# xandergos/terrain-diffusion

Hardware: NVIDIA H100
Metric: denoising steps/sec, 256^2 latent tiles, 30m U-Net (higher is better)
Workload: dtype bf16

## Files before the change

terrain_diffusion_b200/csrc/tdx_igemm.cu:

```cuda
#include "tdx_common.h"
#include "tdx_ptx.cuh"

namespace tdx {

constexpr int kTileH = 16, kTileW = 8;
constexpr int kPatchH = kTileH + 2, kPatchW = kTileW + 2;
constexpr int kKcBytes = kPatchH * kPatchW * 16;
constexpr int kAStageBytes = 8 * kKcBytes;
constexpr int kSA = 3;
constexpr int kMaxSB = 18;
constexpr int kWQ = 2;
constexpr int kEpiWarps = 4 * kWQ;
constexpr int kChunk = 32;
constexpr int kGroups = kChunk / 8;
constexpr int kThreads = 128 + 32 * kEpiWarps;
constexpr int kMaxSplit = 8;
constexpr int kSmemMisc = 14336;
constexpr int kSmemBudget = 227 * 1024;
constexpr int kStgLd = 132;

struct FastDiv {
  uint32_t d, magic;
};
static FastDiv make_fastdiv(int d) {
  FastDiv f;
  f.d = (uint32_t)d;
  f.magic = d <= 1 ? 0u : (uint32_t)(0xFFFFFFFFull / (uint32_t)d + 1ull);
  return f;
}
__device__ __forceinline__ uint32_t fdiv(uint32_t n, const FastDiv& f) { return f.d == 1 ? n : __umulhi(n, f.magic); }

struct IgemmParams {
  int nseg;
  int seg_chunks[3];
  int seg_taps[3];
  const __nv_bfloat16* B;
  int cout, nsplit;
  float inv_cout;
  int ncta;
  int SA;
  int SB;
  int b_stage_bytes;
  int resident;
  int bgroup;
  int ksplit;
  float* ws;
  int H, W, nimg, tiles_x, tiles_y, num_items;
  FastDiv fd_ks, fd_nsplit, fd_per, fd_tx, fd_ty;
  int dtx, dty, dimg;
  int stages_per_item;
  int epi;
  int cluster_stats;
  int xsplit;
  const float* cvec;
  const uint4* resid;
  int resid_spatial, resid_pnorm;
  float resid_scale, clip;
  TdxOutSpec out[3];
  float* rms_out;
  const float* resid_inv;
  unsigned long long* timeline;
  unsigned long long* trace;
};

__device__ __forceinline__ void stage_locate(const IgemmParams& p, int s, int& seg, int& ch, int& tap, int& taps) {
  int base = 0;
  for (seg = 0;; ++seg) {
    taps = p.seg_taps[seg];
    const int n = p.seg_chunks[seg] * taps;
    if (s < base + n || seg == p.nseg - 1) break;
    base += n;
  }
  ch = taps == 9 ? (s - base) / 9 : (s - base);
  tap = (s - base) - ch * taps;
}

#ifndef TDX_DEBUG_HOOKS
#define TDX_DEBUG_HOOKS 0
#endif
#if TDX_DEBUG_HOOKS
#define TDX_TRACE(slot, it)                                                                  \
  do {                                                                                       \
    if (p.trace && blockIdx.x == 0 && (it) < 16) p.trace[(it) * 8 + (slot)] = clock64();     \
  } while (0)
#else
#define TDX_TRACE(slot, it) do { } while (0)
#endif

struct TileWalk {
  int tx, ty, img;
  int dtx, dty, dimg;
  int split, kpart;
  __device__ __forceinline__ void init(const IgemmParams& p) {
    const uint32_t b = blockIdx.x;
    const uint32_t bk = fdiv(b, p.fd_ks);
    kpart = (int)(b - bk * p.fd_ks.d);
    split = (int)(bk - fdiv(bk, p.fd_nsplit) * p.fd_nsplit.d);
    const uint32_t t = fdiv(b, p.fd_per);
    const uint32_t t1 = fdiv(t, p.fd_tx);
    tx = (int)(t - t1 * p.fd_tx.d);
    const uint32_t t2 = fdiv(t1, p.fd_ty);
    ty = (int)(t1 - t2 * p.fd_ty.d);
    img = (int)t2;
    dtx = p.dtx;
    dty = p.dty;
    dimg = p.dimg;
  }
  __device__ __forceinline__ void next(const IgemmParams& p) {
    tx += dtx;
    int c = tx >= p.tiles_x ? 1 : 0;
    tx -= c ? p.tiles_x : 0;
    ty += dty + c;
    c = ty >= p.tiles_y ? 1 : 0;
    ty -= c ? p.tiles_y : 0;
    img += dimg + c;
  }
};
__device__ __forceinline__ void stage_range(const IgemmParams& p, int kpart, int& s0, int& s1) {
  s0 = (int)fdiv((uint32_t)(p.stages_per_item * kpart), p.fd_ks);
  s1 = (int)fdiv((uint32_t)(p.stages_per_item * (kpart + 1)), p.fd_ks);
}

__device__ __forceinline__ uint32_t cluster_ctarank() {
  uint32_t r;
  asm volatile("mov.u32 %0, %%cluster_ctarank;" : "=r"(r));
  return r;
}
__device__ __forceinline__ uint32_t map_to_cta(uint32_t local_smem_addr, uint32_t rank) {
  uint32_t r;
  asm volatile("mapa.shared::cluster.u32 %0, %1, %2;" : "=r"(r) : "r"(local_smem_addr), "r"(rank));
  return r;
}
__device__ __forceinline__ void st_cluster_f32(uint32_t addr, float v) {
  asm volatile("st.shared::cluster.f32 [%0], %1;" ::"r"(addr), "f"(v) : "memory");
}
__device__ __forceinline__ void mbar_arrive_cluster(uint32_t remote_bar_addr) {
  asm volatile("mbarrier.arrive.release.cluster.shared::cluster.b64 _, [%0];" ::"r"(remote_bar_addr) : "memory");
}
__device__ __forceinline__ bool mbar_try_wait_cluster(uint64_t* bar, uint32_t parity) {
  uint32_t ok;
  asm volatile(
      "{\n\t"
      ".reg .pred P;\n\t"
      "mbarrier.try_wait.parity.acquire.cluster.shared::cta.b64 P, [%1], %2;\n\t"
      "selp.b32 %0, 1, 0, P;\n\t"
      "}\n"
      : "=r"(ok)
      : "r"(smem_u32(bar)), "r"(parity)
      : "memory");
  return ok != 0;
}
__device__ __forceinline__ void cluster_sync_all() {
  asm volatile("barrier.cluster.arrive.release.aligned;\n\tbarrier.cluster.wait.acquire.aligned;" ::: "memory");
}

__device__ __forceinline__ void load_acc(const float* stg, int m, int col, float (&v)[kChunk]) {
#pragma unroll
  for (int i = 0; i < kChunk; ++i) v[i] = stg[(col + i) * kStgLd + m];
}

__device__ __forceinline__ float inv_rms(float sumsq, float inv_n) {
  float s;
  asm("sqrt.approx.f32 %0, %1;" : "=f"(s) : "f"(sumsq * inv_n));
  return __fdividef(1.0f, 1e-4f + s);
}

__device__ __forceinline__ void store_chunk(uint4* dst, uint32_t plane, int Wo, int kind, int spatial, bool active,
                                            const float (&v)[kChunk], float hs, float hsk) {
  uint4 u[kGroups];
  if (kind == TDX_OUT_RAW) {
#pragma unroll
    for (int g = 0; g < kGroups; ++g) {
      u[g].x = pack_bf16x2(v[g * 8 + 0], v[g * 8 + 1]);
      u[g].y = pack_bf16x2(v[g * 8 + 2], v[g * 8 + 3]);
      u[g].z = pack_bf16x2(v[g * 8 + 4], v[g * 8 + 5]);
      u[g].w = pack_bf16x2(v[g * 8 + 6], v[g * 8 + 7]);
    }
  } else {
#pragma unroll
    for (int g = 0; g < kGroups; ++g) {
      float w[8];
#pragma unroll
      for (int i = 0; i < 8; ++i) w[i] = mp_silu_scaled(v[g * 8 + i], hs, hsk);
      u[g].x = pack_bf16x2(w[0], w[1]);
      u[g].y = pack_bf16x2(w[2], w[3]);
      u[g].z = pack_bf16x2(w[4], w[5]);
      u[g].w = pack_bf16x2(w[6], w[7]);
    }
  }
  if (!active) return;
  if (spatial == TDX_SP_UP2) {
#pragma unroll
    for (int g = 0; g < kGroups; ++g) {
      uint4* d = dst + (size_t)g * plane;
      d[0] = u[g];
      d[1] = u[g];
      d[Wo] = u[g];
      d[Wo + 1] = u[g];
    }
  } else {
#pragma unroll
    for (int g = 0; g < kGroups; ++g) dst[(size_t)g * plane] = u[g];
  }
}

struct ConsumerRing {
  int sa, sb;
  uint32_t pha;
  uint32_t fmask;
};

template <int kN>
__device__ __forceinline__ void mma_item(const IgemmParams& p, const uint8_t* a_ring, const uint8_t* b_ring,
                                         uint64_t* a_full, uint64_t* a_empty, uint64_t* b_full, uint64_t* b_empty,
                                         ConsumerRing& r, int s0, int s1, bool steady, float* stg) {
  const int lane = threadIdx.x & 31, wl = (threadIdx.x >> 5) & 3, wg = (int)(threadIdx.x >> 7) - 1;
  float acc[kN / 2];
#pragma unroll
  for (int i = 0; i < kN / 2; ++i) acc[i] = 0.f;
  constexpr uint32_t b_lbo = kN * 16;
  const uint32_t a_base = smem_u32(a_ring) + wg * 8 * kPatchW * 16;
  const uint32_t b_base = smem_u32(b_ring);
  const bool deep = p.SB > 1 || p.resident;
  int pend_a = -1, pend_b = -1;
  auto release = [&](int a, int b) {
    __syncwarp();
    if (lane == 0) {
      if (b >= 0) mbar_arrive(&b_empty[b]);
      if (a >= 0) mbar_arrive(&a_empty[a]);
    }
  };
  for (int s = s0; s < s1;) {
    int seg, ch, tap0, taps;
    stage_locate(p, s, seg, ch, tap0, taps);
    const int tap1 = (taps - tap0 < s1 - s) ? taps : tap0 + (s1 - s);
    const int nt = tap1 - tap0;
    s += nt;
    mbar_wait(&a_full[r.sa], r.pha);
    const uint32_t a_stage = a_base + r.sa * kAStageBytes;
    unsigned long long tt = taps == 9 ? (0x16ad18b50820ull >> (5 * tap0)) : (unsigned long long)(kPatchW + 1);
    const int gsz = steady ? nt : p.bgroup;
    int t = 0;
    for (int g0 = 0; g0 < nt; g0 += gsz) {
      const int gn = nt - g0 < gsz ? nt - g0 : gsz;
      if (!steady) {
        mbar_wait(&b_full[r.sb], (r.fmask >> r.sb) & 1u);
        r.fmask ^= 1u << r.sb;
      }
      for (int k = 0; k < gn; ++k, ++t, tt >>= 5) {
        const uint32_t al = a_stage + (uint32_t)(tt & 31ull) * 16;
        const uint32_t bl = b_base + r.sb * p.b_stage_bytes;
        wgmma_fence();
#pragma unroll
        for (int j = 0; j < 4; ++j)
          wgmma_bf16<kN>(acc, make_smem_desc(al + j * 2 * kKcBytes, kKcBytes, kPatchW * 16),
                         make_smem_desc(bl + j * 2 * b_lbo, b_lbo, 128), 1u);
        wgmma_commit();
        const int rel_b = p.resident ? -1 : r.sb;
        const int rel_a = t == nt - 1 ? r.sa : -1;
        if (deep) {
          wgmma_wait<1>();
          release(pend_a, pend_b);
          pend_a = rel_a;
          pend_b = rel_b;
        } else {
          wgmma_wait<0>();
          release(rel_a, rel_b);
        }
        if (++r.sb == p.SB) r.sb = 0;
      }
    }
    if (++r.sa == p.SA) { r.sa = 0; r.pha ^= 1; }
  }
  wgmma_wait<0>();
  release(pend_a, pend_b);
  named_bar_sync(13, 32 * kEpiWarps);
  float* dst = stg + 64 * wg + 16 * wl + (lane >> 2);
#pragma unroll
  for (int j = 0; j < kN / 8; ++j)
#pragma unroll
    for (int i = 0; i < 2; ++i)
#pragma unroll
      for (int c = 0; c < 2; ++c) dst[(8 * j + 2 * (lane & 3) + c) * kStgLd + 8 * i] = acc[4 * j + 2 * i + c];
  named_bar_sync(13, 32 * kEpiWarps);
}

template <bool kCL, int kN>
__global__ void __launch_bounds__(kThreads, 1)
igemm_kernel(const __grid_constant__ CUtensorMap tm0, const __grid_constant__ CUtensorMap tm1,
             const __grid_constant__ CUtensorMap tm2, const __grid_constant__ IgemmParams p) {
  extern __shared__ __align__(1024) uint8_t smem[];
  const int ksplit_ = kCL ? p.ksplit : 1;
  const bool cstats_ = kCL && p.cluster_stats;
  uint8_t* a_ring = smem;
  uint8_t* b_ring = smem + p.SA * kAStageBytes;
  uint64_t* bars = reinterpret_cast<uint64_t*>(b_ring + p.SB * p.b_stage_bytes);
  uint64_t* a_full = bars;
  uint64_t* a_empty = a_full + kSA;
  uint64_t* b_full = a_empty + kSA;
  uint64_t* b_empty = b_full + kMaxSB;
  uint64_t* x_full = b_empty + kMaxSB;
  float* ssq = reinterpret_cast<float*>(bars) + 256;
  float* rss = ssq + 512;
  float* stot = rss + 512;
  float* xstat = stot + 128;
  float* stg = reinterpret_cast<float*>(reinterpret_cast<uint8_t*>(bars) + kSmemMisc);

  const int warp = __shfl_sync(0xffffffffu, threadIdx.x >> 5, 0);
  const int lane = threadIdx.x & 31;
#if TDX_DEBUG_HOOKS
  if (p.trace && blockIdx.x == 0 && threadIdx.x == 0) p.trace[126] = clock64();
  if (p.timeline && threadIdx.x == 0) {
    unsigned long long t;
    asm volatile("mov.u64 %0, %globaltimer;" : "=l"(t));
    atomicMin(p.timeline, t);
  }
#endif

  if (warp == 0 && elect_one()) {
    tma_prefetch_desc(&tm0);
    if (p.nseg > 1) tma_prefetch_desc(&tm1);
    if (p.nseg > 2) tma_prefetch_desc(&tm2);
  }
  if (warp == 2) {
    constexpr int kBars = 2 * kSA + 2 * kMaxSB + 2;
    static_assert(kBars <= 64, "two barriers per lane");
    const int x_full0 = 2 * kSA + 2 * kMaxSB;
#pragma unroll
    for (int k = 0; k < 2; ++k) {
      const int i = lane + 32 * k;
      if (i < kBars) {
        uint32_t count = 1;
        if ((i >= kSA && i < 2 * kSA) || (i >= 2 * kSA + kMaxSB && i < x_full0)) count = kEpiWarps;
        if (i >= x_full0) count = p.xsplit > 1 ? (uint32_t)(p.xsplit - 1) * 128u : 1u;
        mbar_init(&bars[i], count);
      }
    }
    fence_mbar_init();
  }
  __syncthreads();
  if (cstats_) cluster_sync_all();
#if TDX_DEBUG_HOOKS
  if (p.trace && blockIdx.x == 0 && threadIdx.x == 0) p.trace[127] = clock64();
#endif
  pdl_launch_dependents();

  if (warp == 0) {
    pdl_wait();
    int sa = 0;
    uint32_t ph = 0;
    int it = 0;
    TileWalk tw;
    tw.init(p);
    int s0, s1;
    stage_range(p, tw.kpart, s0, s1);
    for (int item = blockIdx.x; item < p.num_items; item += gridDim.x, ++it, tw.next(p)) {
      const int img = tw.img, Y0 = tw.ty * kTileH, X0 = tw.tx * kTileW;
      if (lane == 0) TDX_TRACE(0, it);
      for (int s = s0; s < s1;) {
        int seg, ch, tap, taps;
        stage_locate(p, s, seg, ch, tap, taps);
        const CUtensorMap* tm = seg == 0 ? &tm0 : (seg == 1 ? &tm1 : &tm2);
        mbar_wait(&a_empty[sa], ph ^ 1);
        if (elect_one()) {
          mbar_expect_tx(&a_full[sa], kAStageBytes);
          tma_load_4d(tm, &a_full[sa], a_ring + sa * kAStageBytes, (X0 - 1) * 8, Y0 - 1, ch * 8, img);
        }
        __syncwarp();
        if (++sa == p.SA) { sa = 0; ph ^= 1; }
        s += taps - tap;
      }
    }
    if (ksplit_ > 1) cluster_sync_all();
  } else if (warp == 1) {
    int sb = 0;
    uint32_t ph = 0;
    TileWalk tw;
    tw.init(p);
    const int split = tw.split;
    int st0, st1;
    stage_range(p, tw.kpart, st0, st1);
    for (int item = blockIdx.x; item < p.num_items; item += gridDim.x) {
      const uint8_t* bsrc = reinterpret_cast<const uint8_t*>(p.B) +
                            ((size_t)split * p.stages_per_item + st0) * p.b_stage_bytes;
      if (p.bgroup == 1) {
        for (int ks = 0; ks < st1 - st0; ++ks) {
          mbar_wait(&b_empty[sb], ph ^ 1);
          if (elect_one()) {
            mbar_expect_tx(&b_full[sb], p.b_stage_bytes);
            bulk_load_1d(bsrc + (size_t)ks * p.b_stage_bytes, &b_full[sb], b_ring + sb * p.b_stage_bytes,
                         p.b_stage_bytes);
          }
          __syncwarp();
          if (++sb == p.SB) { sb = 0; ph ^= 1; }
        }
        continue;
      }
      int ks = 0;
      for (int s = st0; s < st1;) {
        int seg, ch, tap0, taps;
        stage_locate(p, s, seg, ch, tap0, taps);
        const int nt = (taps - tap0 < st1 - s) ? taps - tap0 : st1 - s;
        int head = sb, gi = 0;
        for (int t = 0; t < nt; ++t) {
          if (!p.resident) mbar_wait(&b_empty[sb], ph ^ 1);
          const bool first = gi == 0;
          if (++gi == p.bgroup) gi = 0;
          if (first) head = sb;
          if (elect_one()) {
            uint64_t* full = &b_full[head];
            if (first) mbar_expect_tx(full, (uint32_t)(nt - t < p.bgroup ? nt - t : p.bgroup) * p.b_stage_bytes);
            bulk_load_1d(bsrc + (size_t)(ks + t) * p.b_stage_bytes, full, b_ring + sb * p.b_stage_bytes,
                         p.b_stage_bytes);
          }
          __syncwarp();
          if (++sb == p.SB) { sb = 0; ph ^= 1; }
        }
        ks += nt;
        s += nt;
      }
      if (p.resident) break;
    }
    if (ksplit_ > 1) cluster_sync_all();
  } else if (warp < 4) {
    if (ksplit_ > 1) cluster_sync_all();
  } else {
    pdl_wait();
    const int q = warp & 3;
    const int wq = (warp - 4) >> 2;
    const int m = q * 32 + lane;
    const int y = m >> 3, x = m & 7;
    const int C8 = p.cout >> 3;
    const bool need_norm = (p.epi & TDX_EPI_PNORM) || p.out[0].kind == TDX_OUT_PNORM_SILU ||
                           p.out[1].kind == TDX_OUT_PNORM_SILU || p.out[2].kind == TDX_OUT_PNORM_SILU ||
                           p.rms_out != nullptr;
    const uint32_t my_rank = cstats_ ? cluster_ctarank() : 0;
    TileWalk tw;
    tw.init(p);
    ConsumerRing ring = {0, 0, 0u, 0u};
    int s0, s1;
    stage_range(p, tw.kpart, s0, s1);
    const int ks = ksplit_, kpart = tw.kpart;
    const int slice = p.ncta / ks, sch = slice / kChunk;
    const int nchunks_all = p.ncta / kChunk;
    const int nchunks = sch;
    const int col0 = kpart * slice;
    const int chbase = tw.split * p.ncta + col0;
    const uint32_t plane = (uint32_t)(p.H * p.W);
    struct OffSpec {
      uint32_t istride, rowstep, colstep, tpart;
    };
    auto make_spec = [&](int spatial, uint32_t planes_per_img) -> OffSpec {
      OffSpec o;
      if (spatial == TDX_SP_DOWN2) {
        o.istride = planes_per_img * (plane >> 2);
        o.rowstep = (uint32_t)(kTileH / 2) * (uint32_t)(p.W >> 1);
        o.colstep = kTileW / 2;
        o.tpart = (uint32_t)((y >> 1) * (p.W >> 1) + (x >> 1));
      } else if (spatial == TDX_SP_UP2) {
        o.istride = planes_per_img * (plane << 2);
        o.rowstep = (uint32_t)(kTileH * 2) * (uint32_t)(p.W << 1);
        o.colstep = kTileW * 2;
        o.tpart = (uint32_t)((y << 1) * (p.W << 1) + (x << 1));
      } else {
        o.istride = planes_per_img * plane;
        o.rowstep = (uint32_t)kTileH * (uint32_t)p.W;
        o.colstep = kTileW;
        o.tpart = (uint32_t)(y * p.W + x);
      }
      return o;
    };
    auto item_off = [&](const OffSpec& o, const TileWalk& t) -> uint32_t {
      return (uint32_t)t.img * o.istride + (uint32_t)t.ty * o.rowstep + (uint32_t)t.tx * o.colstep + o.tpart;
    };
    const bool has_resid = (p.epi & TDX_EPI_RESID) != 0;
    const uint32_t rplane = p.resid_spatial == TDX_SP_UP2 ? (plane >> 2) : (p.resid_spatial == TDX_SP_DOWN2 ? (plane << 2) : plane);
    const int rsp = p.resid_spatial == TDX_SP_UP2 ? TDX_SP_DOWN2 : (p.resid_spatial == TDX_SP_DOWN2 ? TDX_SP_UP2 : TDX_SP_SAME);
    const OffSpec rspec = make_spec(rsp, (uint32_t)C8), rinv_spec = make_spec(rsp, 1u);
    OffSpec ospec[3];
    uint32_t omask = 0;
#pragma unroll
    for (int o = 0; o < 3; ++o) {
      const int sp = p.out[o].spatial;
      ospec[o] = make_spec(sp, (uint32_t)C8);
      const uint32_t oplane = sp == TDX_SP_DOWN2 ? (plane >> 2) : (sp == TDX_SP_UP2 ? (plane << 2) : plane);
      ospec[o].tpart += (uint32_t)(chbase >> 3) * oplane;
      omask |= (uint32_t)(p.out[o].kind != TDX_OUT_NONE && !(sp == TDX_SP_DOWN2 && ((y | x) & 1))) << o;
    }
    constexpr int kPreN = (kChunk / 4 > kGroups) ? kChunk / 4 : kGroups;
    uint4 pre[kPreN];
    const uint4* rbase_pre = nullptr;
    float rinv_pre = 1.f;
    const bool cv_ahead = (p.epi & TDX_EPI_EMB_SILU) && !has_resid;
    const bool ahead = has_resid || cv_ahead;
    const bool own_rnorm = has_resid && p.resid_pnorm && !p.resid_inv;
    auto fetch_ahead = [&](const TileWalk& t) {
      if (cv_ahead) {
        const uint4* cp = reinterpret_cast<const uint4*>(p.cvec + (size_t)t.img * p.cout + chbase + wq * kChunk);
#pragma unroll
        for (int j = 0; j < kChunk / 4; ++j) pre[j] = (wq < nchunks) ? __ldg(cp + j) : make_uint4(0, 0, 0, 0);
        return;
      }
      if (!has_resid) return;
      const int Y_ = t.ty * kTileH + y, X_ = t.tx * kTileW + x;
      const bool vld = (Y_ < p.H) && (X_ < p.W);
      rbase_pre = p.resid + item_off(rspec, t);
      if (p.resid_inv) rinv_pre = vld ? __ldg(p.resid_inv + item_off(rinv_spec, t)) : 0.f;
      const uint4* rptr = rbase_pre + (size_t)((chbase >> 3) + wq * kGroups) * rplane;
#pragma unroll
      for (int g = 0; g < kGroups; ++g)
        pre[g] = (vld && wq < nchunks) ? __ldg(rptr + (size_t)g * rplane) : make_uint4(0, 0, 0, 0);
    };
    if (ahead) fetch_ahead(tw);
    int it = 0;
    for (int item = blockIdx.x; item < p.num_items; item += gridDim.x, ++it, tw.next(p)) {
      const int img = tw.img;
      const int Y = tw.ty * kTileH + y, X = tw.tx * kTileW + x;
      const bool valid = (Y < p.H) && (X < p.W);
      if (warp == 4 && lane == 0) TDX_TRACE(1, it);
      mma_item<kN>(p, a_ring, b_ring, a_full, a_empty, b_full, b_empty, ring, s0, s1, p.resident && it > 0, stg);
      if (warp == 4 && lane == 0) TDX_TRACE(2, it);

      const float* red_src = nullptr;
      if (ks > 1) {
        float* wsg = p.ws + (size_t)fdiv((uint32_t)item, p.fd_ks) * (ks - 1) * p.ncta * 128;
        if (warp == 4 && lane == 0) TDX_TRACE(3, it);
        for (int ck = wq; ck < nchunks_all; ck += kWQ) {
          const int dst = ck / sch;
          if (dst == kpart) continue;
          const int slot = kpart - (kpart > dst ? 1 : 0);
          float* d = wsg + ((size_t)(dst * (ks - 1) + slot) * slice + (size_t)(ck - dst * sch) * kChunk) * 128 + m;
          float v[kChunk];
          __syncwarp();
          load_acc(stg, m, ck * kChunk, v);
#pragma unroll
          for (int j = 0; j < kChunk; ++j) __stcg(d + (size_t)j * 128, v[j]);
        }
        cluster_sync_all();
        red_src = wsg + (size_t)kpart * (ks - 1) * slice * 128 + m;
      }
      const float* cvb = p.cvec ? p.cvec + (size_t)img * p.cout + chbase : nullptr;
      auto add_partials = [&](int ck, float (&v)[kChunk]) {
        for (int kp = 0; kp < ks - 1; ++kp) {
          const float* src = red_src + ((size_t)kp * slice + (size_t)(ck * kChunk)) * 128;
#pragma unroll
          for (int j = 0; j < kChunk; ++j) v[j] += __ldcg(src + (size_t)j * 128);
        }
      };

      {
        float rscale = p.resid_scale;
        const uint4* rbase = rbase_pre;
        const bool more = ahead && item + (int)gridDim.x < p.num_items;
        TileWalk tn = tw;
        tn.next(p);
        if (has_resid && p.resid_inv) {
          rscale = p.resid_scale * rinv_pre;
        } else if (own_rnorm) {
          float ss = 0.f;
          auto sq8 = [&](const uint4& u) {
            float a, b;
            unpack_bf16x2(u.x, a, b); ss = fmaf(a, a, fmaf(b, b, ss));
            unpack_bf16x2(u.y, a, b); ss = fmaf(a, a, fmaf(b, b, ss));
            unpack_bf16x2(u.z, a, b); ss = fmaf(a, a, fmaf(b, b, ss));
            unpack_bf16x2(u.w, a, b); ss = fmaf(a, a, fmaf(b, b, ss));
          };
          if (valid) {
            for (int g0 = wq * 2; g0 < C8; g0 += 2 * kWQ) {
              const uint4 u0 = __ldg(rbase + (size_t)g0 * rplane), u1 = __ldg(rbase + (size_t)(g0 + 1) * rplane);
              sq8(u0);
              sq8(u1);
            }
          }
          rss[wq * 128 + m] = ss;
          named_bar_sync(9 + q, 32 * kWQ);
          ss = 0.f;
#pragma unroll
          for (int w = 0; w < kWQ; ++w) ss += rss[w * 128 + m];
          rscale = p.resid_scale * inv_rms(ss, p.inv_cout);
        }
        uint4* optr[3];
        bool oact[3];
#pragma unroll
        for (int o = 0; o < 3; ++o) {
          oact[o] = valid && ((omask >> o) & 1u);
          optr[o] = reinterpret_cast<uint4*>(p.out[o].ptr) + item_off(ospec[o], tw);
        }


        auto compute_v = [&](int ck, float (&v)[kChunk]) {
          __syncwarp();
          load_acc(stg, m, col0 + ck * kChunk, v);
          add_partials(ck, v);
          if (p.epi & TDX_EPI_EMB_SILU) {
#pragma unroll
            for (int i = 0; i < kChunk; i += 4) {
              const uint4 cu = (cv_ahead && ck == wq) ? pre[i >> 2] : __ldg(reinterpret_cast<const uint4*>(cvb + ck * kChunk + i));
              const float4 c4 = make_float4(__uint_as_float(cu.x), __uint_as_float(cu.y), __uint_as_float(cu.z), __uint_as_float(cu.w));
              v[i + 0] = mp_silu_f(v[i + 0] * c4.x);
              v[i + 1] = mp_silu_f(v[i + 1] * c4.y);
              v[i + 2] = mp_silu_f(v[i + 2] * c4.z);
              v[i + 3] = mp_silu_f(v[i + 3] * c4.w);
            }
          }
          if (p.epi & TDX_EPI_RESID) {
            const uint4* rptr = rbase + (size_t)((chbase >> 3) + ck * kGroups) * rplane;
#pragma unroll
            for (int g = 0; g < kGroups; ++g) {
              uint4 u = (ck == wq) ? pre[g] : (valid ? __ldg(rptr + (size_t)g * rplane) : make_uint4(0, 0, 0, 0));
              float rr[8];
              unpack_bf16x2(u.x, rr[0], rr[1]);
              unpack_bf16x2(u.y, rr[2], rr[3]);
              unpack_bf16x2(u.z, rr[4], rr[5]);
              unpack_bf16x2(u.w, rr[6], rr[7]);
#pragma unroll
              for (int i = 0; i < 8; ++i) v[g * 8 + i] = fmaf(rscale, rr[i], v[g * 8 + i]);
            }
          }
          if (p.clip > 0.f) {
#pragma unroll
            for (int i = 0; i < kChunk; ++i) v[i] = fminf(fmaxf(v[i], -p.clip), p.clip);
          }
        };
        auto emit_v = [&](int ck, float (&v)[kChunk], float inv) {
          if (p.epi & TDX_EPI_PNORM) {
#pragma unroll
            for (int i = 0; i < kChunk; ++i) v[i] *= inv;
          }
#pragma unroll
          for (int o = 0; o < 3; ++o) {
            const int kind = p.out[o].kind, sp = p.out[o].spatial;
            if (kind == TDX_OUT_NONE) continue;
            float hs = 0.5f * p.out[o].scale;
            if (kind == TDX_OUT_PNORM_SILU) hs = (p.epi & TDX_EPI_PNORM) ? 0.5f : 0.5f * inv;
            const uint32_t oplane = sp == TDX_SP_DOWN2 ? (plane >> 2) : (sp == TDX_SP_UP2 ? (plane << 2) : plane);
            const int Wo = sp == TDX_SP_DOWN2 ? (p.W >> 1) : (sp == TDX_SP_UP2 ? (p.W << 1) : p.W);
            store_chunk(optr[o] + (size_t)(ck * kGroups) * oplane, oplane, Wo, kind, sp, oact[o], v, hs,
                        hs * (1.0f / 0.596f));
          }
        };
        auto finish_norm = [&](float sumsq) -> float {
          ssq[wq * 128 + m] = sumsq;
          named_bar_sync(1 + q, 32 * kWQ);
          float tot = 0.f;
#pragma unroll
          for (int w = 0; w < kWQ; ++w) tot += ssq[w * 128 + m];
          if (cstats_) {
            const int par = it & 1;
            if (wq == 0) {
              for (uint32_t r = 0; r < (uint32_t)p.xsplit; ++r) {
                if (r == my_rank) continue;
                st_cluster_f32(map_to_cta(smem_u32(&xstat[(par * kMaxSplit + my_rank) * 128 + m]), r), tot);
                mbar_arrive_cluster(map_to_cta(smem_u32(&x_full[par]), r));
              }
              const uint32_t xph = (it >> 1) & 1;
              if (!mbar_try_wait_cluster(&x_full[par], xph)) {
                const long long t0 = clock64();
                while (!mbar_try_wait_cluster(&x_full[par], xph)) {
                  if (clock64() - t0 > TDX_WAIT_LIMIT) asm volatile("trap;");
                }
              }
              for (uint32_t r = 0; r < (uint32_t)p.xsplit; ++r)
                if (r != my_rank) tot += xstat[(par * kMaxSplit + r) * 128 + m];
              stot[m] = tot;
            }
            named_bar_sync(5 + q, 32 * kWQ);
            tot = stot[m];
          }
          return inv_rms(tot, p.inv_cout);
        };

        float v[kChunk];
        float sumsq = 0.f, inv = 1.f;
        const bool reuse = need_norm && nchunks <= kWQ;
#pragma unroll 1
        for (int pass = need_norm ? 0 : 1; pass < 2; ++pass) {
#pragma unroll 1
          for (int ck = wq; ck < nchunks; ck += kWQ) {
            if (pass == 0 || !reuse) {
              compute_v(ck, v);
              if (ck == wq && (reuse || pass == 1) && more) fetch_ahead(tn);
            }
            if (pass == 0) {
#pragma unroll
              for (int i = 0; i < kChunk; ++i) sumsq = fmaf(v[i], v[i], sumsq);
            } else {
              emit_v(ck, v, inv);
            }
          }
          if (pass == 0) {
            inv = finish_norm(sumsq);
            if (p.rms_out && wq == 0 && kpart == 0 && tw.split == 0 && valid)
              p.rms_out[(uint32_t)img * plane + (uint32_t)(Y * p.W + X)] = inv;
          }
        }
      }
      if (warp == 4 && lane == 0) TDX_TRACE(4, it);
    }
  }

  __syncthreads();
  if (cstats_) cluster_sync_all();
#if TDX_DEBUG_HOOKS
  if (p.trace && blockIdx.x == 0 && threadIdx.x == 96) p.trace[125] = clock64();
  if (p.timeline && threadIdx.x == 0) {
    unsigned long long t;
    asm volatile("mov.u64 %0, %globaltimer;" : "=l"(t));
    atomicMax(p.timeline + 1, t);
  }
#endif
}

static unsigned long long* g_trace_ptr = nullptr;
static unsigned long long* g_timeline_ptr = nullptr;
static int g_timeline_idx = 0, g_timeline_cap = 0;

static int ensure_scratch(float** ws);

typedef decltype(&igemm_kernel<false, 64>) IgemmKernel;

static IgemmKernel igemm_kernel_for(bool cluster, int n) {
  switch (n) {
    case 64: return cluster ? igemm_kernel<true, 64> : igemm_kernel<false, 64>;
    case 128: return cluster ? igemm_kernel<true, 128> : igemm_kernel<false, 128>;
    case 192: return cluster ? igemm_kernel<true, 192> : igemm_kernel<false, 192>;
    default: return cluster ? igemm_kernel<true, 256> : igemm_kernel<false, 256>;
  }
}

int igemm_prepare() {
  static bool seen[16] = {false};
  if (first_use_on_device(seen)) {
    for (int n = 64; n <= 256; n += 64)
      for (int cl = 0; cl < 2; ++cl)
        TDX_CHECK_CUDA(
            cudaFuncSetAttribute(igemm_kernel_for(cl, n), cudaFuncAttributeMaxDynamicSharedMemorySize, kSmemBudget));
  }
  float* ws;
  return ensure_scratch(&ws);
}

static bool needs_norm(const TdxIgemmDesc& d) {
  if (d.epi_flags & TDX_EPI_PNORM) return true;
  if (d.rms_out) return true;
  for (int o = 0; o < 3; ++o)
    if (d.out[o].kind == TDX_OUT_PNORM_SILU) return true;
  return false;
}

constexpr size_t kWsBytes = 24u << 20;
static float* g_ws[16] = {nullptr};

static int ensure_scratch(float** ws) {
  int dev = 0;
  TDX_CHECK_CUDA(cudaGetDevice(&dev));
  TDX_REQUIRE(dev >= 0 && dev < 16, "igemm: device index %d out of range", dev);
  if (!g_ws[dev]) TDX_CHECK_CUDA(cudaMalloc(&g_ws[dev], kWsBytes));
  *ws = g_ws[dev];
  return TDX_OK;
}

static int max_active_clusters(int csize) {
  static int cache[9] = {0};
  if (csize <= 1) return sm_count();
  if (csize > 8) return 0;
  if (cache[csize]) return cache[csize];
  cudaLaunchConfig_t cfg;
  memset(&cfg, 0, sizeof(cfg));
  cudaLaunchAttribute attr[1];
  cfg.gridDim = dim3((sm_count() / csize) * csize);
  cfg.blockDim = dim3(kThreads);
  cfg.dynamicSmemBytes = kSmemBudget;
  attr[0].id = cudaLaunchAttributeClusterDimension;
  attr[0].val.clusterDim.x = csize;
  attr[0].val.clusterDim.y = 1;
  attr[0].val.clusterDim.z = 1;
  cfg.attrs = attr;
  cfg.numAttrs = 1;
  int n = 0;
  cudaFuncSetAttribute(igemm_kernel<true, 64>, cudaFuncAttributeMaxDynamicSharedMemorySize, kSmemBudget);
  if (cudaOccupancyMaxActiveClusters(&n, igemm_kernel<true, 64>, &cfg) != cudaSuccess || n <= 0) {
    cudaGetLastError();
    n = (sm_count() * 3 / 4) / csize;
  }
  cache[csize] = n;
  return n;
}

struct ItemShape { int ncta, resident, sa, sb, ksplit; };

static ItemShape choose_item_shape(int cout, int tiles, int stages, int chunks, int forced_n, bool norm) {
  if (forced_n && (forced_n > cout || cout % forced_n)) forced_n = 0;
  double best = 1e30;
  ItemShape bs = {64, 0, kSA, 2, 1};
  for (int n = 64; n <= 256 && n <= cout; n += 64) {
    if (cout % n) continue;
    if (forced_n && n != forced_n) continue;
    const int nsplit = cout / n;
    if (norm && nsplit > kMaxSplit) continue;
    const int stage_bytes = n * 128;
    const int free_bytes = kSmemBudget - kSmemMisc - n * kStgLd * 4;
    const int sa = free_bytes - kSA * kAStageBytes >= 2 * stage_bytes ? kSA : 2;
    const int ring_budget = free_bytes - sa * kAStageBytes;
    const long items = (long)tiles * nsplit;
    for (int ks = 1; ks <= 8; ++ks) {
      const int csize = ks * ((norm && nsplit > 1) ? nsplit : 1);
      if (ks > 1) {
        if (n % (kChunk * ks) || ks > stages || csize > kMaxSplit) continue;
        if (items * ks > (long)max_active_clusters(csize) * csize) continue;
        if ((size_t)items * (ks - 1) * n * 512 > kWsBytes) continue;
      }
      const int my_stages = (stages + ks - 1) / ks;
      const int my_chunks = (chunks + ks - 1) / ks + (ks > 1 ? 1 : 0);
      const int resident = (ks == 1 && stages * stage_bytes <= ring_budget && stages <= kMaxSB) ? 1 : 0;
      int sb = resident ? stages : ring_budget / stage_bytes;
      if (sb > kMaxSB) sb = kMaxSB;
      if (sb < 1) continue;
      int grid = items * ks < sm_count() ? (int)(items * ks) : sm_count();
      grid -= grid % (nsplit * ks);
      if (grid <= 0) continue;
      const double rounds = (double)((items * ks + grid - 1) / grid);
      const double mma = rounds * my_stages * 4.0 * n * (sb < 2 && !resident ? 2.0 : 1.0) + 800.0;
      const double a_bytes = (double)items * ks * my_chunks * kAStageBytes;
      const double b_bytes = resident ? (double)grid * stages * stage_bytes : (double)items * stages * stage_bytes;
      const double red_bytes = ks > 1 ? (double)(ks - 1) / ks * n * 512.0 : 0.0;
      const double l2 = (a_bytes + b_bytes + 2.0 * red_bytes * items * ks) / 5000.0;
      const double per_sm = (double)(my_chunks * kAStageBytes + my_stages * stage_bytes) / 56.0;
      const int epi_chunks = ((n / ks) / kChunk + 3) / 4;
      const double epi = rounds * epi_chunks * 100.0;
      const double red = ks > 1 ? 2.0 * red_bytes / 56.0 + 2000.0 : 0.0;
      double t = mma;
      if (l2 > t) t = l2;
      if (per_sm > t) t = per_sm;
      t += epi + red;
      if (t < best) { best = t; bs = {n, resident, sa, sb, ks}; }
    }
  }
  return bs;
}

int igemm_launch(const TdxIgemmDesc& d, const CUtensorMap* tms, cudaStream_t stream) {
  IgemmParams p;
  memset(&p, 0, sizeof(p));
  p.nseg = d.n_seg;
  p.stages_per_item = 0;
  int chunks = 0;
  for (int s = 0; s < d.n_seg; ++s) {
    p.seg_chunks[s] = d.a_channels[s] / 64;
    p.seg_taps[s] = d.a_taps[s];
    p.stages_per_item += p.seg_chunks[s] * p.seg_taps[s];
    chunks += p.seg_chunks[s];
  }
  p.B = reinterpret_cast<const __nv_bfloat16*>(d.b_packed);
  p.cout = d.c_out;
  p.inv_cout = 1.0f / (float)d.c_out;
  p.H = d.height;
  p.W = d.width;
  p.nimg = d.n_img;
  p.tiles_x = (d.width + kTileW - 1) / kTileW;
  p.tiles_y = (d.height + kTileH - 1) / kTileH;
  const int tiles = p.tiles_x * p.tiles_y * d.n_img;
  const bool norm = needs_norm(d);
  const ItemShape shp = choose_item_shape(d.c_out, tiles, p.stages_per_item, chunks, d.n_per_item, norm);
  p.ncta = shp.ncta;
  p.resident = shp.resident;
  p.SA = shp.sa;
  p.SB = shp.sb;
  p.bgroup = (shp.resident || shp.sb >= 18) ? 9 : 1;
  p.ksplit = shp.ksplit;
  p.nsplit = d.c_out / p.ncta;
  p.b_stage_bytes = p.ncta * 128;
  p.num_items = tiles * p.nsplit * p.ksplit;
  if (p.ksplit > 1) {
    int rc_ws = ensure_scratch(&p.ws);
    if (rc_ws != TDX_OK) return rc_ws;
  }
  p.epi = d.epi_flags;
  p.cluster_stats = (norm && p.nsplit * p.ksplit > 1) ? 1 : 0;
  p.xsplit = p.cluster_stats ? p.nsplit * p.ksplit : 1;
  const int cluster = p.cluster_stats ? p.xsplit : p.ksplit;
  p.cvec = d.cvec;
  p.resid = reinterpret_cast<const uint4*>(d.resid);
  p.resid_spatial = d.resid_spatial;
  p.resid_pnorm = d.resid_pnorm;
  p.resid_scale = d.resid_scale;
  p.clip = d.clip;
  for (int o = 0; o < 3; ++o) p.out[o] = d.out[o];
  p.rms_out = d.rms_out;
  p.resid_inv = d.resid_inv;
  p.trace = g_trace_ptr;
  p.timeline = (g_timeline_ptr && g_timeline_idx < g_timeline_cap) ? g_timeline_ptr + 2 * (g_timeline_idx++) : nullptr;

  int rc_prep = igemm_prepare();
  if (rc_prep != TDX_OK) return rc_prep;
  int grid = p.num_items < sm_count() ? p.num_items : sm_count();
  grid -= grid % (p.nsplit * p.ksplit);
  {
    const int per = p.nsplit * p.ksplit;
    p.fd_ks = make_fastdiv(p.ksplit);
    p.fd_nsplit = make_fastdiv(p.nsplit);
    p.fd_per = make_fastdiv(per);
    p.fd_tx = make_fastdiv(p.tiles_x);
    p.fd_ty = make_fastdiv(p.tiles_y);
    int dstep = grid / per;
    p.dtx = dstep % p.tiles_x;
    dstep /= p.tiles_x;
    p.dty = dstep % p.tiles_y;
    p.dimg = dstep / p.tiles_y;
  }
  const int smem = p.SA * kAStageBytes + p.SB * p.b_stage_bytes + kSmemMisc + p.ncta * kStgLd * 4;
  const CUtensorMap& t0 = tms[0];
  const CUtensorMap& t1 = tms[d.n_seg > 1 ? 1 : 0];
  const CUtensorMap& t2 = tms[d.n_seg > 2 ? 2 : 0];
  cudaLaunchConfig_t cfg;
  cudaLaunchAttribute attr[2];
  fill_launch_config(&cfg, attr, dim3(grid), dim3(kThreads), smem < 120 * 1024 ? 120 * 1024 : smem, stream);
  if (cluster > 1) {
    attr[cfg.numAttrs].id = cudaLaunchAttributeClusterDimension;
    attr[cfg.numAttrs].val.clusterDim.x = cluster;
    attr[cfg.numAttrs].val.clusterDim.y = 1;
    attr[cfg.numAttrs].val.clusterDim.z = 1;
    cfg.attrs = attr;
    cfg.numAttrs += 1;
  }
  TDX_CHECK_CUDA(cudaLaunchKernelEx(&cfg, igemm_kernel_for(cluster > 1, p.ncta), t0, t1, t2, p));
  return TDX_OK;
}

int igemm_validate(const TdxIgemmDesc& d) {
  TDX_REQUIRE(d.n_seg >= 1 && d.n_seg <= 3, "igemm: n_seg=%d not in 1..3", d.n_seg);
  for (int s = 0; s < d.n_seg; ++s) {
    TDX_REQUIRE(d.a_ptr[s] != nullptr, "igemm: a_ptr[%d] is null", s);
    TDX_REQUIRE(d.a_channels[s] > 0 && d.a_channels[s] % 64 == 0, "igemm: a_channels[%d]=%d not a multiple of 64", s,
                d.a_channels[s]);
    TDX_REQUIRE(d.a_taps[s] == 9 || d.a_taps[s] == 1, "igemm: a_taps[%d]=%d not 9 or 1", s, d.a_taps[s]);
  }
  TDX_REQUIRE(d.b_packed != nullptr, "igemm: b_packed is null");
  TDX_REQUIRE(d.c_out >= 64 && d.c_out <= 2048 && d.c_out % 64 == 0, "igemm: c_out=%d must be a multiple of 64 <= 2048",
              d.c_out);
  if (needs_norm(d))
    TDX_REQUIRE(d.c_out / d.n_per_item <= kMaxSplit, "igemm: pixel-norm over %d channels needs n_per_item >= %d",
                d.c_out, d.c_out / kMaxSplit);
  TDX_REQUIRE(d.n_per_item >= 64 && d.n_per_item <= 256 && d.n_per_item % 64 == 0 && d.c_out % d.n_per_item == 0,
              "igemm: n_per_item=%d must be 64/128/192/256 and divide c_out=%d (use tdx_igemm_choose_n)", d.n_per_item,
              d.c_out);
  TDX_REQUIRE((unsigned long long)d.n_img * (d.c_out / 8) * d.height * d.width * 4ull < (1ull << 32),
              "igemm: tensor of %d x %d x %d x %d exceeds the 32-bit element offsets of the epilogue", d.n_img, d.c_out,
              d.height, d.width);
  TDX_REQUIRE(d.n_img >= 1 && d.height >= 8 && d.width >= 8 && d.height % 8 == 0 && d.width % 8 == 0,
              "igemm: bad shape n=%d h=%d w=%d (h, w multiples of 8)", d.n_img, d.height, d.width);
  if (d.epi_flags & TDX_EPI_EMB_SILU) TDX_REQUIRE(d.cvec != nullptr, "igemm: EMB_SILU needs cvec");
  if (d.resid_inv)
    TDX_REQUIRE((d.epi_flags & TDX_EPI_RESID) && !d.resid_pnorm,
                "igemm: resid_inv needs TDX_EPI_RESID and resid_pnorm == 0 (it replaces the recomputed pixel-norm)");
  if (d.epi_flags & TDX_EPI_RESID) {
    TDX_REQUIRE(d.resid != nullptr, "igemm: RESID needs resid");
    if (d.resid_spatial == TDX_SP_UP2)
      TDX_REQUIRE(d.height % 2 == 0 && d.width % 2 == 0, "igemm: UP2 residual needs even h, w");
  }
  for (int o = 0; o < 3; ++o) {
    if (d.out[o].kind == TDX_OUT_NONE) continue;
    TDX_REQUIRE(d.out[o].ptr != nullptr, "igemm: out[%d].ptr is null", o);
    TDX_REQUIRE(d.out[o].kind >= 1 && d.out[o].kind <= 3, "igemm: out[%d].kind=%d", o, d.out[o].kind);
    if (d.out[o].spatial == TDX_SP_DOWN2)
      TDX_REQUIRE(d.height % 2 == 0 && d.width % 2 == 0, "igemm: DOWN2 output needs even h, w");
  }
  return TDX_OK;
}

}

extern "C" void tdx_debug_set_igemm_trace(void* device_u64x128) {
  tdx::g_trace_ptr = reinterpret_cast<unsigned long long*>(device_u64x128);
}
extern "C" void tdx_debug_set_igemm_timeline(void* device_u64_pairs, int capacity) {
  tdx::g_timeline_ptr = reinterpret_cast<unsigned long long*>(device_u64_pairs);
  tdx::g_timeline_idx = 0;
  tdx::g_timeline_cap = capacity;
}

extern "C" int tdx_igemm_choose_n(int32_t c_out, int32_t n_img, int32_t height, int32_t width,
                                  const int32_t* a_channels, const int32_t* a_taps, int32_t n_seg) {
  if (c_out < 64 || c_out % 64 || n_seg < 1 || n_seg > 3) return 64;
  int stages = 0, chunks = 0;
  for (int s = 0; s < n_seg; ++s) {
    stages += (a_channels[s] / 64) * a_taps[s];
    chunks += a_channels[s] / 64;
  }
  const int tiles = ((width + tdx::kTileW - 1) / tdx::kTileW) * ((height + tdx::kTileH - 1) / tdx::kTileH) * n_img;
  return tdx::choose_item_shape(c_out, tiles, stages, chunks, 0, true).ncta;
}

extern "C" void tdx_debug_igemm_plan(int32_t c_out, int32_t n_img, int32_t height, int32_t width,
                                     const int32_t* a_channels, const int32_t* a_taps, int32_t n_seg,
                                     int32_t n_per_item, int32_t needs_norm, int32_t* out4) {
  int stages = 0, chunks = 0;
  for (int s = 0; s < n_seg; ++s) {
    stages += (a_channels[s] / 64) * a_taps[s];
    chunks += a_channels[s] / 64;
  }
  const int tiles = ((width + tdx::kTileW - 1) / tdx::kTileW) * ((height + tdx::kTileH - 1) / tdx::kTileH) * n_img;
  tdx::ItemShape shp = tdx::choose_item_shape(c_out, tiles, stages, chunks, n_per_item, needs_norm != 0);
  out4[0] = shp.ncta; out4[1] = shp.ksplit; out4[2] = shp.resident; out4[3] = shp.sb;
}

extern "C" int64_t tdx_igemm_packed_weight_elems(const int32_t* a_channels, const int32_t* a_taps, int32_t n_seg,
                                                 int32_t c_out) {
  int64_t n = 0;
// ... 20 lines not shown
```

Baseline: 670.3.

## Add dedicated epilogue warpgroup overlapping MMA with epilogue via staging barriers

Adds a kernel variant with a separate 128-thread epilogue warpgroup, so the 8 MMA warps can start the next item's wgmma while the epilogue drains the staged accumulators. The two sides hand off through stg_full/stg_empty mbarriers, and setmaxnreg moves registers from producers and MMA warps to the epilogue. With a single epilogue warpgroup, the norm reductions skip cross-warp named barriers, and residual loads are prefetched one chunk ahead. The variant is chosen heuristically for ncta<=128 and long items. The costs are a single staging buffer shared between the two sides, extra smem round trips for the norm pass, and register pressure with a 128-register cap on the MMA warps.

After: 687.1, median of 6. 1.03x the previous value.

```diff
diff --git a/terrain_diffusion_b200/csrc/tdx_igemm.cu b/terrain_diffusion_b200/csrc/tdx_igemm.cu
--- a/terrain_diffusion_b200/csrc/tdx_igemm.cu
+++ b/terrain_diffusion_b200/csrc/tdx_igemm.cu
@@ -9,11 +9,10 @@
 constexpr int kAStageBytes = 8 * kKcBytes;
 constexpr int kSA = 3;
 constexpr int kMaxSB = 18;
-constexpr int kWQ = 2;
-constexpr int kEpiWarps = 4 * kWQ;
+constexpr int kMmaWarps = 8;
 constexpr int kChunk = 32;
 constexpr int kGroups = kChunk / 8;
-constexpr int kThreads = 128 + 32 * kEpiWarps;
+constexpr int block_threads(bool epi_wg) { return epi_wg ? 512 : 384; }
 constexpr int kMaxSplit = 8;
 constexpr int kSmemMisc = 14336;
 constexpr int kSmemBudget = 227 * 1024;
@@ -121,6 +120,11 @@
   s1 = (int)fdiv((uint32_t)(p.stages_per_item * (kpart + 1)), p.fd_ks);
 }
 
+template <int kRegs>
+__device__ __forceinline__ void setmaxnreg_dec() { asm volatile("setmaxnreg.dec.sync.aligned.u32 %0;" ::"n"(kRegs)); }
+template <int kRegs>
+__device__ __forceinline__ void setmaxnreg_inc() { asm volatile("setmaxnreg.inc.sync.aligned.u32 %0;" ::"n"(kRegs)); }
+
 __device__ __forceinline__ uint32_t cluster_ctarank() {
   uint32_t r;
   asm volatile("mov.u32 %0, %%cluster_ctarank;" : "=r"(r));
@@ -159,6 +163,11 @@
   for (int i = 0; i < kChunk; ++i) v[i] = stg[(col + i) * kStgLd + m];
 }
 
+__device__ __forceinline__ void store_acc(float* stg, int m, int col, const float (&v)[kChunk]) {
+#pragma unroll
+  for (int i = 0; i < kChunk; ++i) stg[(col + i) * kStgLd + m] = v[i];
+}
+
 __device__ __forceinline__ float inv_rms(float sumsq, float inv_n) {
   float s;
   asm("sqrt.approx.f32 %0, %1;" : "=f"(s) : "f"(sumsq * inv_n));
@@ -210,10 +219,11 @@
   uint32_t fmask;
 };
 
-template <int kN>
+template <int kN, bool kEW>
 __device__ __forceinline__ void mma_item(const IgemmParams& p, const uint8_t* a_ring, const uint8_t* b_ring,
                                          uint64_t* a_full, uint64_t* a_empty, uint64_t* b_full, uint64_t* b_empty,
-                                         ConsumerRing& r, int s0, int s1, bool steady, float* stg) {
+                                         ConsumerRing& r, int s0, int s1, bool steady, float* stg,
+                                         uint64_t* stg_full, uint64_t* stg_empty, int it) {
   const int lane = threadIdx.x & 31, wl = (threadIdx.x >> 5) & 3, wg = (int)(threadIdx.x >> 7) - 1;
   float acc[kN / 2];
 #pragma unroll
@@ -274,7 +284,8 @@
   }
   wgmma_wait<0>();
   release(pend_a, pend_b);
-  named_bar_sync(13, 32 * kEpiWarps);
+  if (kEW) mbar_wait(stg_empty, (uint32_t)(it & 1) ^ 1u);
+  else named_bar_sync(13, 32 * kMmaWarps);
   float* dst = stg + 64 * wg + 16 * wl + (lane >> 2);
 #pragma unroll
   for (int j = 0; j < kN / 8; ++j)
@@ -282,16 +293,21 @@
     for (int i = 0; i < 2; ++i)
 #pragma unroll
       for (int c = 0; c < 2; ++c) dst[(8 * j + 2 * (lane & 3) + c) * kStgLd + 8 * i] = acc[4 * j + 2 * i + c];
-  named_bar_sync(13, 32 * kEpiWarps);
-}
-
-template <bool kCL, int kN>
-__global__ void __launch_bounds__(kThreads, 1)
+  if (kEW) mbar_arrive(stg_full);
+  else named_bar_sync(13, 32 * kMmaWarps);
+}
+
+template <bool kCL, int kN, bool kEW>
+__global__ void __launch_bounds__(block_threads(kEW), 1)
 igemm_kernel(const __grid_constant__ CUtensorMap tm0, const __grid_constant__ CUtensorMap tm1,
              const __grid_constant__ CUtensorMap tm2, const __grid_constant__ IgemmParams p) {
   extern __shared__ __align__(1024) uint8_t smem[];
   const int ksplit_ = kCL ? p.ksplit : 1;
   const bool cstats_ = kCL && p.cluster_stats;
+  constexpr bool kEpiWG = kEW;
+  static_assert(!kEW || kN <= 128, "wider accumulators do not fit the consumers' 128 registers");
+  constexpr int kWQ = kEpiWG ? 1 : 2;
+  constexpr int kEpiWarp0 = kEpiWG ? 12 : 4;
   uint8_t* a_ring = smem;
   uint8_t* b_ring = smem + p.SA * kAStageBytes;
   uint64_t* bars = reinterpret_cast<uint64_t*>(b_ring + p.SB * p.b_stage_bytes);
@@ -300,6 +316,8 @@
   uint64_t* b_full = a_empty + kSA;
   uint64_t* b_empty = b_full + kMaxSB;
   uint64_t* x_full = b_empty + kMaxSB;
+  uint64_t* stg_full = x_full + 2;
+  uint64_t* stg_empty = stg_full + 1;
   float* ssq = reinterpret_cast<float*>(bars) + 256;
   float* rss = ssq + 512;
   float* stot = rss + 512;
@@ -323,16 +341,18 @@
     if (p.nseg > 2) tma_prefetch_desc(&tm2);
   }
   if (warp == 2) {
-    constexpr int kBars = 2 * kSA + 2 * kMaxSB + 2;
-    static_assert(kBars <= 64, "two barriers per lane");
-    const int x_full0 = 2 * kSA + 2 * kMaxSB;
+    constexpr int kBars = 2 * kSA + 2 * kMaxSB + 4;
+    static_assert(kBars <= 64 && kBars * 8 <= 256 * 4, "two barriers per lane, below the statistics arrays");
+    const int x_full0 = 2 * kSA + 2 * kMaxSB, stg0 = x_full0 + 2;
 #pragma unroll
     for (int k = 0; k < 2; ++k) {
       const int i = lane + 32 * k;
       if (i < kBars) {
         uint32_t count = 1;
-        if ((i >= kSA && i < 2 * kSA) || (i >= 2 * kSA + kMaxSB && i < x_full0)) count = kEpiWarps;
-        if (i >= x_full0) count = p.xsplit > 1 ? (uint32_t)(p.xsplit - 1) * 128u : 1u;
+        if ((i >= kSA && i < 2 * kSA) || (i >= 2 * kSA + kMaxSB && i < x_full0)) count = kMmaWarps;
+        if (i >= x_full0 && i < stg0) count = p.xsplit > 1 ? (uint32_t)(p.xsplit - 1) * 128u : 1u;
+        if (i == stg0) count = 32 * kMmaWarps;
+        if (i == stg0 + 1) count = 128;
         mbar_init(&bars[i], count);
       }
     }
@@ -346,6 +366,7 @@
   pdl_launch_dependents();
 
   if (warp == 0) {
+    if (kEpiWG) setmaxnreg_dec<56>();
     pdl_wait();
     int sa = 0;
     uint32_t ph = 0;
@@ -373,6 +394,7 @@
     }
     if (ksplit_ > 1) cluster_sync_all();
   } else if (warp == 1) {
+    if (kEpiWG) setmaxnreg_dec<56>();
     int sb = 0;
     uint32_t ph = 0;
     TileWalk tw;
@@ -423,11 +445,27 @@
     }
     if (ksplit_ > 1) cluster_sync_all();
   } else if (warp < 4) {
+    if (kEpiWG) setmaxnreg_dec<56>();
+    if (ksplit_ > 1) cluster_sync_all();
+  } else if (kEpiWG && warp < kEpiWarp0) {
+    TileWalk tw;
+    tw.init(p);
+    ConsumerRing ring = {0, 0, 0u, 0u};
+    int s0, s1;
+    stage_range(p, tw.kpart, s0, s1);
+    int it = 0;
+    for (int item = blockIdx.x; item < p.num_items; item += gridDim.x, ++it) {
+      if (warp == 4 && lane == 0) TDX_TRACE(1, it);
+      mma_item<kN, kEW>(p, a_ring, b_ring, a_full, a_empty, b_full, b_empty, ring, s0, s1, p.resident && it > 0, stg,
+                   stg_full, stg_empty, it);
+      if (warp == 4 && lane == 0) TDX_TRACE(2, it);
+    }
     if (ksplit_ > 1) cluster_sync_all();
   } else {
+    if (kEpiWG) setmaxnreg_inc<200>();
     pdl_wait();
     const int q = warp & 3;
-    const int wq = (warp - 4) >> 2;
+    const int wq = (warp - kEpiWarp0) >> 2;
     const int m = q * 32 + lane;
     const int y = m >> 3, x = m & 7;
     const int C8 = p.cout >> 3;
@@ -517,14 +555,20 @@
       const int img = tw.img;
       const int Y = tw.ty * kTileH + y, X = tw.tx * kTileW + x;
       const bool valid = (Y < p.H) && (X < p.W);
-      if (warp == 4 && lane == 0) TDX_TRACE(1, it);
-      mma_item<kN>(p, a_ring, b_ring, a_full, a_empty, b_full, b_empty, ring, s0, s1, p.resident && it > 0, stg);
-      if (warp == 4 && lane == 0) TDX_TRACE(2, it);
+      if (kEpiWG) {
+        mbar_wait(stg_full, (uint32_t)it & 1u);
+        if (warp == kEpiWarp0 && lane == 0) TDX_TRACE(5, it);
+      } else {
+        if (warp == 4 && lane == 0) TDX_TRACE(1, it);
+        mma_item<kN, kEW>(p, a_ring, b_ring, a_full, a_empty, b_full, b_empty, ring, s0, s1, p.resident && it > 0, stg,
+                     stg_full, stg_empty, it);
+        if (warp == 4 && lane == 0) TDX_TRACE(2, it);
+      }
 
       const float* red_src = nullptr;
       if (ks > 1) {
         float* wsg = p.ws + (size_t)fdiv((uint32_t)item, p.fd_ks) * (ks - 1) * p.ncta * 128;
-        if (warp == 4 && lane == 0) TDX_TRACE(3, it);
+        if (warp == kEpiWarp0 && lane == 0) TDX_TRACE(3, it);
         for (int ck = wq; ck < nchunks_all; ck += kWQ) {
           const int dst = ck / sch;
           if (dst == kpart) continue;
@@ -557,26 +601,45 @@
         if (has_resid && p.resid_inv) {
           rscale = p.resid_scale * rinv_pre;
         } else if (own_rnorm) {
-          float ss = 0.f;
-          auto sq8 = [&](const uint4& u) {
+          auto sq8 = [](float& ss, const uint4& u) {
             float a, b;
             unpack_bf16x2(u.x, a, b); ss = fmaf(a, a, fmaf(b, b, ss));
             unpack_bf16x2(u.y, a, b); ss = fmaf(a, a, fmaf(b, b, ss));
             unpack_bf16x2(u.z, a, b); ss = fmaf(a, a, fmaf(b, b, ss));
             unpack_bf16x2(u.w, a, b); ss = fmaf(a, a, fmaf(b, b, ss));
           };
-          if (valid) {
-            for (int g0 = wq * 2; g0 < C8; g0 += 2 * kWQ) {
-              const uint4 u0 = __ldg(rbase + (size_t)g0 * rplane), u1 = __ldg(rbase + (size_t)(g0 + 1) * rplane);
-              sq8(u0);
-              sq8(u1);
+          float ss = 0.f;
+          if constexpr (kWQ == 1) {
+            float ss1 = 0.f;
+            if (valid) {
+              for (int g0 = 0; g0 < C8; g0 += 8) {
+                uint4 u[8];
+#pragma unroll
+                for (int g = 0; g < 8; ++g) u[g] = __ldg(rbase + (size_t)(g0 + g) * rplane);
+#pragma unroll
+                for (int g = 0; g < 8; g += 4) {
+                  sq8(ss, u[g]);
+                  sq8(ss, u[g + 1]);
+                  sq8(ss1, u[g + 2]);
+                  sq8(ss1, u[g + 3]);
+                }
+              }
             }
+            ss += ss1;
+          } else {
+            if (valid) {
+              for (int g0 = wq * 2; g0 < C8; g0 += 2 * kWQ) {
+                const uint4 u0 = __ldg(rbase + (size_t)g0 * rplane), u1 = __ldg(rbase + (size_t)(g0 + 1) * rplane);
+                sq8(ss, u0);
+                sq8(ss, u1);
+              }
+            }
+            rss[wq * 128 + m] = ss;
+            named_bar_sync(9 + q, 32 * kWQ);
+            ss = 0.f;
+#pragma unroll
+            for (int w = 0; w < kWQ; ++w) ss += rss[w * 128 + m];
           }
-          rss[wq * 128 + m] = ss;
-          named_bar_sync(9 + q, 32 * kWQ);
-          ss = 0.f;
-#pragma unroll
-          for (int w = 0; w < kWQ; ++w) ss += rss[w * 128 + m];
           rscale = p.resid_scale * inv_rms(ss, p.inv_cout);
         }
         uint4* optr[3];
@@ -588,6 +651,7 @@
         }
 
 
+        uint4 rnext[kGroups];
         auto compute_v = [&](int ck, float (&v)[kChunk]) {
           __syncwarp();
           load_acc(stg, m, col0 + ck * kChunk, v);
@@ -605,9 +669,20 @@
           }
           if (p.epi & TDX_EPI_RESID) {
             const uint4* rptr = rbase + (size_t)((chbase >> 3) + ck * kGroups) * rplane;
+            uint4 cur[kGroups];
 #pragma unroll
             for (int g = 0; g < kGroups; ++g) {
-              uint4 u = (ck == wq) ? pre[g] : (valid ? __ldg(rptr + (size_t)g * rplane) : make_uint4(0, 0, 0, 0));
+              if (kWQ == 1) cur[g] = ck == wq ? pre[g] : rnext[g];
+              else cur[g] = (ck == wq) ? pre[g] : (valid ? __ldg(rptr + (size_t)g * rplane) : make_uint4(0, 0, 0, 0));
+            }
+            if (kWQ == 1 && ck + 1 < nchunks) {
+#pragma unroll
+              for (int g = 0; g < kGroups; ++g)
+                rnext[g] = valid ? __ldg(rptr + (size_t)(kGroups + g) * rplane) : make_uint4(0, 0, 0, 0);
+            }
+#pragma unroll
+            for (int g = 0; g < kGroups; ++g) {
+              const uint4 u = cur[g];
               float rr[8];
               unpack_bf16x2(u.x, rr[0], rr[1]);
               unpack_bf16x2(u.y, rr[2], rr[3]);
@@ -639,12 +714,16 @@
                         hs * (1.0f / 0.596f));
           }
         };
-        auto finish_norm = [&](float sumsq) -> float {
-          ssq[wq * 128 + m] = sumsq;
-          named_bar_sync(1 + q, 32 * kWQ);
+        auto finish_norm = [&](float sq0, float sq1) -> float {
           float tot = 0.f;
-#pragma unroll
-          for (int w = 0; w < kWQ; ++w) tot += ssq[w * 128 + m];
+          if constexpr (kWQ == 1) {
+            tot = sq0 + sq1;
+          } else {
+            ssq[wq * 128 + m] = sq0;
+            named_bar_sync(1 + q, 32 * kWQ);
+#pragma unroll
+            for (int w = 0; w < kWQ; ++w) tot += ssq[w * 128 + m];
+          }
           if (cstats_) {
             const int par = it & 1;
             if (wq == 0) {
@@ -662,40 +741,51 @@
               }
               for (uint32_t r = 0; r < (uint32_t)p.xsplit; ++r)
                 if (r != my_rank) tot += xstat[(par * kMaxSplit + r) * 128 + m];
-              stot[m] = tot;
+              if (kWQ > 1) stot[m] = tot;
             }
-            named_bar_sync(5 + q, 32 * kWQ);
-            tot = stot[m];
+            if (kWQ > 1) {
+              named_bar_sync(5 + q, 32 * kWQ);
+              tot = stot[m];
+            }
           }
           return inv_rms(tot, p.inv_cout);
         };
 
         float v[kChunk];
-        float sumsq = 0.f, inv = 1.f;
+        float sq0 = 0.f, sq1 = 0.f, inv = 1.f;
         const bool reuse = need_norm && nchunks <= kWQ;
+        const bool keep = kEpiWG && need_norm && !reuse;
 #pragma unroll 1
         for (int pass = need_norm ? 0 : 1; pass < 2; ++pass) {
 #pragma unroll 1
           for (int ck = wq; ck < nchunks; ck += kWQ) {
-            if (pass == 0 || !reuse) {
+            if (pass == 0 || !(reuse || keep)) {
               compute_v(ck, v);
-              if (ck == wq && (reuse || pass == 1) && more) fetch_ahead(tn);
+              if (ck == wq && (reuse || keep || pass == 1) && more) fetch_ahead(tn);
+              if (keep) store_acc(stg, m, col0 + ck * kChunk, v);
+            } else if (keep) {
+              __syncwarp();
+              load_acc(stg, m, col0 + ck * kChunk, v);
             }
             if (pass == 0) {
-#pragma unroll
-              for (int i = 0; i < kChunk; ++i) sumsq = fmaf(v[i], v[i], sumsq);
+              float sq = (kWQ == 1 && (ck & 1)) ? sq1 : sq0;
+#pragma unroll
+              for (int i = 0; i < kChunk; ++i) sq = fmaf(v[i], v[i], sq);
+              if (kWQ == 1 && (ck & 1)) sq1 = sq;
+              else sq0 = sq;
             } else {
               emit_v(ck, v, inv);
             }
           }
           if (pass == 0) {
-            inv = finish_norm(sumsq);
+            inv = finish_norm(sq0, sq1);
             if (p.rms_out && wq == 0 && kpart == 0 && tw.split == 0 && valid)
               p.rms_out[(uint32_t)img * plane + (uint32_t)(Y * p.W + X)] = inv;
           }
         }
       }
-      if (warp == 4 && lane == 0) TDX_TRACE(4, it);
+      if (kEpiWG) mbar_arrive(stg_empty);
+      if (warp == kEpiWarp0 && lane == 0) TDX_TRACE(4, it);
     }
   }
 
@@ -717,14 +807,18 @@
 
 static int ensure_scratch(float** ws);
 
-typedef decltype(&igemm_kernel<false, 64>) IgemmKernel;
-
-static IgemmKernel igemm_kernel_for(bool cluster, int n) {
+typedef decltype(&igemm_kernel<false, 64, false>) IgemmKernel;
+
+static IgemmKernel igemm_kernel_for(bool cluster, int n, bool ew) {
   switch (n) {
-    case 64: return cluster ? igemm_kernel<true, 64> : igemm_kernel<false, 64>;
-    case 128: return cluster ? igemm_kernel<true, 128> : igemm_kernel<false, 128>;
-    case 192: return cluster ? igemm_kernel<true, 192> : igemm_kernel<false, 192>;
-    default: return cluster ? igemm_kernel<true, 256> : igemm_kernel<false, 256>;
+    case 64:
+      if (ew) return cluster ? igemm_kernel<true, 64, true> : igemm_kernel<false, 64, true>;
+      return cluster ? igemm_kernel<true, 64, false> : igemm_kernel<false, 64, false>;
+    case 128:
+      if (ew) return cluster ? igemm_kernel<true, 128, true> : igemm_kernel<false, 128, true>;
+      return cluster ? igemm_kernel<true, 128, false> : igemm_kernel<false, 128, false>;
+    case 192: return cluster ? igemm_kernel<true, 192, false> : igemm_kernel<false, 192, false>;
+    default: return cluster ? igemm_kernel<true, 256, false> : igemm_kernel<false, 256, false>;
   }
 }
 
@@ -733,8 +827,9 @@
   if (first_use_on_device(seen)) {
     for (int n = 64; n <= 256; n += 64)
       for (int cl = 0; cl < 2; ++cl)
-        TDX_CHECK_CUDA(
-            cudaFuncSetAttribute(igemm_kernel_for(cl, n), cudaFuncAttributeMaxDynamicSharedMemorySize, kSmemBudget));
+        for (int ew = 0; ew < (n <= 128 ? 2 : 1); ++ew)
+          TDX_CHECK_CUDA(cudaFuncSetAttribute(igemm_kernel_for(cl, n, ew), cudaFuncAttributeMaxDynamicSharedMemorySize,
+                                              kSmemBudget));
   }
   float* ws;
   return ensure_scratch(&ws);
@@ -769,7 +864,7 @@
   memset(&cfg, 0, sizeof(cfg));
   cudaLaunchAttribute attr[1];
   cfg.gridDim = dim3((sm_count() / csize) * csize);
-  cfg.blockDim = dim3(kThreads);
+  cfg.blockDim = dim3(block_threads(true));
   cfg.dynamicSmemBytes = kSmemBudget;
   attr[0].id = cudaLaunchAttributeClusterDimension;
   attr[0].val.clusterDim.x = csize;
@@ -778,8 +873,8 @@
   cfg.attrs = attr;
   cfg.numAttrs = 1;
   int n = 0;
-  cudaFuncSetAttribute(igemm_kernel<true, 64>, cudaFuncAttributeMaxDynamicSharedMemorySize, kSmemBudget);
-  if (cudaOccupancyMaxActiveClusters(&n, igemm_kernel<true, 64>, &cfg) != cudaSuccess || n <= 0) {
+  cudaFuncSetAttribute(igemm_kernel<true, 64, true>, cudaFuncAttributeMaxDynamicSharedMemorySize, kSmemBudget);
+  if (cudaOccupancyMaxActiveClusters(&n, igemm_kernel<true, 64, true>, &cfg) != cudaSuccess || n <= 0) {
     cudaGetLastError();
     n = (sm_count() * 3 / 4) / csize;
   }
@@ -909,12 +1004,15 @@
     p.dimg = dstep / p.tiles_y;
   }
   const int smem = p.SA * kAStageBytes + p.SB * p.b_stage_bytes + kSmemMisc + p.ncta * kStgLd * 4;
+  const bool own_rnorm = (d.epi_flags & TDX_EPI_RESID) && d.resid_pnorm && !d.resid_inv;
+  const bool epi_wg = p.ncta <= 128 && p.num_items >= 2 * grid &&
+                      p.stages_per_item * p.ncta >= (own_rnorm ? 1152 : 576);
   const CUtensorMap& t0 = tms[0];
   const CUtensorMap& t1 = tms[d.n_seg > 1 ? 1 : 0];
   const CUtensorMap& t2 = tms[d.n_seg > 2 ? 2 : 0];
   cudaLaunchConfig_t cfg;
   cudaLaunchAttribute attr[2];
-  fill_launch_config(&cfg, attr, dim3(grid), dim3(kThreads), smem < 120 * 1024 ? 120 * 1024 : smem, stream);
+  fill_launch_config(&cfg, attr, dim3(grid), dim3(block_threads(epi_wg)), smem < 120 * 1024 ? 120 * 1024 : smem, stream);
   if (cluster > 1) {
     attr[cfg.numAttrs].id = cudaLaunchAttributeClusterDimension;
     attr[cfg.numAttrs].val.clusterDim.x = cluster;
@@ -923,7 +1021,7 @@
     cfg.attrs = attr;
     cfg.numAttrs += 1;
   }
-  TDX_CHECK_CUDA(cudaLaunchKernelEx(&cfg, igemm_kernel_for(cluster > 1, p.ncta), t0, t1, t2, p));
+  TDX_CHECK_CUDA(cudaLaunchKernelEx(&cfg, igemm_kernel_for(cluster > 1, p.ncta, epi_wg), t0, t1, t2, p));
   return TDX_OK;
 }
 
```
